# fpgasystems/GPU-FPGA-Recommendation-System

Measured on AMD Instinct MI355X. Metric: inferences/sec at batch 256, higher is better.
Workload: dtype f32; 1 GPU; Model-A (embedding_47_krnl: 47 tables, 1.415 GB) batch=256, fp32 FC 352-1024-512-256-1, all tables resident in one GPU's HBM; hash-filled tables, uniform per-table indices; index rows resident in HBM when the timed region starts (1024 rotating buffers), scores left in HBM (the bench contract's definition of `value`); value_pcie_inclusive = the reference's own loop (cuda_server.c:460-461,494-495): ; batch=256, driver_threads=2, workers_per_thread=2, batches_per_launch=64, parallelism=replicas x1

## Files before the change

gpu-fpga-recommendation-system_amd/csrc/fr_fused.hip:

```cpp
#include "fr_device.h"

#ifdef FR_EPI_FORMS
#include <cstdarg>
#include <cstdio>
thread_local char fr_epi_noted[96];
thread_local int fr_epi_hip_error = 0;
void fr_set_error(const char *, ...) {}
void fr_note_kernel(const char *fmt, ...) {
    va_list ap;
    va_start(ap, fmt);
    vsnprintf(fr_epi_noted, sizeof(fr_epi_noted), fmt, ap);
    va_end(ap);
}
#define FR_NO_DEFAULT_FORM() return FR_ERR_INVALID
#else
static int fused_epi_forward(const FrFusedArgs &a, int kind, hipStream_t s) {
    char name[96] = "";
    const int e = fr_epi_fused_launch(&a, kind, s, name, sizeof(name));
    if (e) FR_FAIL(FR_ERR_HIP, "launch of the epilogue form of the fused kernel failed: %s", hipGetErrorString((hipError_t)e));
    fr_note_kernel("%s", name);
    return FR_OK;
}
#endif

// ... 157 lines not shown
    }
}

template <int NB, int IPT, typename Sink>
__device__ __forceinline__ bool ft_gather_tile(const FrFusedArgs &a, const FrFusedBatch &bt, int m0, int wl, int ig, Sink &&sink) {
    uint64_t base[NB];
    uint32_t stride[NB], rows[NB], icol[NB];
    bool dense[NB];
#pragma unroll
    for (int p = 0; p < NB; p++) {
        const int w = 64 * p + wl < a.n_words ? 64 * p + wl : a.n_words - 1;
        const uint4 d0 = reinterpret_cast<const uint4 *>(a.words)[2 * w];
        const uint4 d1 = reinterpret_cast<const uint4 *>(a.words)[2 * w + 1];
        dense[p] = (d0.w & FR_DESC_DENSE) != 0;
        base[p] = (dense[p] ? (uint64_t)reinterpret_cast<uintptr_t>(bt.dense) : 0ull) + (((uint64_t)d0.y << 32) | d0.x);
        stride[p] = d0.z, rows[p] = d1.x, icol[p] = dense[p] ? 0u : d0.w * 4u;
    }
    const __amdgpu_buffer_rsrc_t rs_idx = __builtin_amdgcn_make_buffer_rsrc(const_cast<int32_t *>(bt.idx), 0, (unsigned)bt.batch * (unsigned)a.idx_stride * 4u, 0x00020000);
    uint32_t id[NB][IPT];
#pragma unroll
    for (int p = 0; p < NB; p++)
#pragma unroll
        for (int i = 0; i < IPT; i++)
            id[p][i] = (uint32_t)__builtin_amdgcn_raw_buffer_load_b32(rs_idx, (unsigned)(m0 + IPT * ig + i) * (unsigned)a.idx_stride * 4u + icol[p], 0, 0);
    bool bad = false;
    uint4 v[NB][IPT];
    auto load_rows = [&](int p) {
#pragma unroll
        for (int i = 0; i < IPT; i++) {
            const unsigned m = (unsigned)(m0 + IPT * ig + i);
            uint32_t r = id[p][i];
            const bool oob = !dense[p] & (r >= rows[p]);
            bad |= oob;
            r = oob ? 0u : r;
            r = dense[p] ? (m < (unsigned)bt.batch ? m : 0u) : r;
            typedef const u32x4_t __attribute__((address_space(1))) * gptr_t;
            const u32x4_t q = *(gptr_t)(base[p] + (uint64_t)r * stride[p]);
            v[p][i] = make_uint4(q.x, q.y, q.z, q.w);
        }
    };
    load_rows(0);
#pragma unroll
    for (int p = 0; p < NB; p++) {
        if (p + 1 < NB) load_rows(p + 1);
        const int w = 64 * p + wl;
        if (w < a.n_words) {
#pragma unroll
            for (int i = 0; i < IPT; i++) sink(w, i, (m0 + IPT * ig + i < bt.batch) ? v[p][i] : make_uint4(0u, 0u, 0u, 0u));
        }
    }
    return bad;
}

template <int T2W, int KG, int WPE, bool DB, bool EPI>
__device__ __forceinline__ void fused_tile_body(const FrFusedArgs &a) {
    extern __shared__ uint4 lds[];
    constexpr int RD = (WPE == 2) ? 1 : 2;
    const int KQ = a.K / 4;
    uint4 *Xq = lds;
    uint4 *R1b[2] = {Xq + (size_t)KQ * FR_FT_LD, Xq + (size_t)(KQ + (DB ? 64 : 0)) * FR_FT_LD};
    uint4 *R2 = lds;
    uint4 *R3 = DB ? lds + (size_t)(a.H2 / 4) * FR_FT_LD : lds;
    const int tid = threadIdx.x, lane = tid & 63;
    const int wave = __builtin_amdgcn_readfirstlane(tid >> 6);
    const int hk = lane >> 5, lm = lane & 31;
    const int bi = blockIdx.x / a.tiles_per_batch, tile = blockIdx.x - bi * a.tiles_per_batch;
    const FrFusedBatch &bt = a.b[bi];
    const int m0 = tile * 32;
    if (m0 >= bt.batch) return;
    int n_st = 0;
    auto stamp = [&]() {
        if (a.stamps && tid == 0 && n_st < 14) {
            a.stamps[16ull * blockIdx.x + n_st] = __builtin_amdgcn_s_memrealtime();
            if (n_st == 1) a.stamps[16ull * blockIdx.x + 14] = __builtin_amdgcn_s_memtime();
            if (n_st == 11) a.stamps[16ull * blockIdx.x + 15] = __builtin_amdgcn_s_memtime();
        }
        n_st++;
    };
    auto wstamp = [&](int k) {
        if (a.stamps && lane == 0) a.stamps[16ull * gridDim.x + (8ull * blockIdx.x + wave) * 4 + k] = __builtin_amdgcn_s_memrealtime();
    };
    stamp();
    const FtW W1 = ft_w(a.w1q, a.K, a.H1, hk, lm), W2 = ft_w(a.w2q, a.H1, a.H2, hk, lm), W3 = ft_w(a.w3q, a.H2, a.H3, hk, lm);
    constexpr int RA = 16 / RD, RB = 24 / T2W / RD;
    constexpr int KG1 = KG > 0 ? KG : 1;
    float4 ring1[RA][1];
    if constexpr (KG > 0) ft_ring_fill<1, RA, KG1>(ring1, W1, 32 * wave, 0);

    if constexpr (KG > 0) {
        const int wl = tid & 63, ig = tid >> 6;
        constexpr int NB = (2 * KG1 + 63) / 64;
        const bool bad = ft_gather_tile<NB, 4>(a, bt, m0, wl, ig, [&](int w, int i, const uint4 &x) { Xq[(size_t)w * FR_FT_LD + 4 * ig + i] = x; });
        if (bad) atomicOr_system(a.err_flag, 1);
    } else {
        const int wl = tid & 63, ig = tid >> 6;
        bool bad = false;
        for (int w0 = 0; w0 < a.n_words; w0 += 64) {
            const int w = w0 + wl;
            if (w < a.n_words) {
                const uint4 d0 = reinterpret_cast<const uint4 *>(a.words)[2 * w];
                const uint4 d1 = reinterpret_cast<const uint4 *>(a.words)[2 * w + 1];
                const uint64_t src = ((uint64_t)d0.y << 32) | d0.x;
                const uint32_t stride = d0.z, idx_col = d0.w, rows = d1.x;
                const bool is_dense = (idx_col & FR_DESC_DENSE) != 0;
                const char *base = is_dense ? reinterpret_cast<const char *>(bt.dense) + src : reinterpret_cast<const char *>(src);
                uint32_t id[4];
#pragma unroll
                for (int i = 0; i < 4; i++) {
                    const int m = m0 + 4 * ig + i;
                    id[i] = 0;
                    if (m < bt.batch) id[i] = is_dense ? (uint32_t)m : (uint32_t)bt.idx[(size_t)m * a.idx_stride + idx_col];
                    if (!is_dense && id[i] >= rows) {
                        bad = true;
                        id[i] = 0;
                    }
                }
                uint4 v[4];
#pragma unroll
                for (int i = 0; i < 4; i++) v[i] = *reinterpret_cast<const uint4 *>(base + (uint64_t)id[i] * stride);
#pragma unroll
                for (int i = 0; i < 4; i++)
                    Xq[(size_t)w * FR_FT_LD + 4 * ig + i] = (m0 + 4 * ig + i < bt.batch) ? v[i] : make_uint4(0u, 0u, 0u, 0u);
            }
        }
        if (bad) atomicOr_system(a.err_flag, 1);
    }
    __syncthreads();
    stamp();

    f32x16 acc2[T2W];
#pragma unroll
    for (int t = 0; t < T2W; t++)
#pragma unroll
        for (int i = 0; i < 16; i++) acc2[t][i] = 0.0f;
    const int n_chunks = a.H1 / 256;
    for (int c = 0; c < n_chunks; c++) {
        f32x16 acc1[1];
#pragma unroll
        for (int i = 0; i < 16; i++) acc1[0][i] = 0.0f;
        if constexpr (KG > 0) ft_gemm_ct<1, RA, KG1>(acc1, ring1, W1, c * 256 + 32 * wave, Xq, 0, 0, hk, lm);
        else ft_gemm<1, 4>(acc1, a.w1q, a.H1, c * 256 + 32 * wave, Xq, 0, 0, a.K / 8, hk, lm);
        stamp();
        if (c == 1) wstamp(0);
        if (c == 2) wstamp(3);
        float4 ring2[RB][T2W];
        ft_ring_fill<T2W, RB, 32>(ring2, W2, 32 * T2W * wave, 32 * c);
        uint4 *R1 = R1b[c & 1];
        if (!DB && c > 0) __syncthreads();
        ft_store_tile<EPI>(R1, acc1[0], 32 * wave, hk, lm, a.epi[0], c * 256 + 32 * wave);
        __syncthreads();
        stamp();
        if (c == 1) wstamp(1);
        ft_gemm_ct<T2W, RB, 32>(acc2, ring2, W2, 32 * T2W * wave, R1, 0, 32 * c, hk, lm);
        if (c == 1) wstamp(2);
        if constexpr (KG > 0) {
            const int cn = (c + 1 < n_chunks) ? c + 1 : c;
            ft_ring_fill<1, RA, KG1>(ring1, W1, cn * 256 + 32 * wave, 0);
        }
    }
    float4 ring3[RA][1];
    ft_ring_fill<1, RA, 32 * T2W>(ring3, W3, 32 * wave, 0);
    __syncthreads();
#pragma unroll
    for (int t = 0; t < T2W; t++) ft_store_tile<EPI>(R2, acc2[t], 32 * (T2W * wave + t), hk, lm, a.epi[1], 32 * (T2W * wave + t));
    __syncthreads();
    stamp();

    f32x16 acc3[1];
#pragma unroll
    for (int i = 0; i < 16; i++) acc3[0][i] = 0.0f;
    ft_gemm_ct<1, RA, 32 * T2W>(acc3, ring3, W3, 32 * wave, R2, 0, 0, hk, lm);
    if (!DB) __syncthreads();
    ft_store_tile<EPI>(R3, acc3[0], 32 * wave, hk, lm, a.epi[2], 32 * wave);
    __syncthreads();
    stamp();
    {
        const int il = tid & 31, sl = tid >> 5;
        const int rows_per = (a.H3 / 4) / 16;
        float s = 0.0f;
        for (int q = sl * rows_per; q < (sl + 1) * rows_per; q++) {
            const uint4 r = R3[(size_t)q * FR_FT_LD + il];
            const float4 w4 = reinterpret_cast<const float4 *>(a.wout)[q];
            s = fmaf(w4.x, __uint_as_float(r.x), s);
            s = fmaf(w4.y, __uint_as_float(r.y), s);
            s = fmaf(w4.z, __uint_as_float(r.z), s);
            s = fmaf(w4.w, __uint_as_float(r.w), s);
        }
        float *part = reinterpret_cast<float *>(R3 + (size_t)64 * FR_FT_LD);
        part[sl * 32 + il] = s;
        __syncthreads();
        if (tid < 32 && m0 + tid < bt.batch) {
            float t = part[tid];
#pragma unroll
            for (int i = 1; i < 16; i++) t += part[i * 32 + tid];
            t = ft_out_bias<EPI>(a, t);
            bt.scores[m0 + tid] = t;
        }
    }
    stamp();
}

#ifndef FR_EPI_FORMS
template <int T2W, int KG, int WPE, bool DB>
__global__ void __launch_bounds__(512, WPE) fr_fused_tile_kernel(const FrFusedArgs a) {
    fused_tile_body<T2W, KG, WPE, DB, false>(a);
}
#else
template <int T2W, int KG, int WPE, bool DB>
__global__ void __launch_bounds__(512, WPE) fr_epi_tile_kernel(const FrFusedArgs a) {
    fused_tile_body<T2W, KG, WPE, DB, true>(a);
}
#endif

size_t frk_fused_lds_bytes(int K, int H2, int wpe) {
    if (wpe == 4) {
        const size_t phase1 = (size_t)(K / 4) + 64, phase2 = (size_t)(H2 / 4) > 68 ? (size_t)(H2 / 4) : 68;
        return (phase1 > phase2 ? phase1 : phase2) * FR_FT_LD * 16;
    }
    const size_t phase1 = (size_t)(K / 4) + 128;
    const size_t phase2 = (size_t)(H2 / 4) + 64 + 4;
    return (phase1 > phase2 ? phase1 : phase2) * FR_FT_LD * 16;
}

bool frk_fused_ok(int K, int H1, int H2, int H3) {
    const bool straight = (K == 352 || K == 880) && H2 == 512;
    if ((!straight && K % 32) || H1 % 256 || (H2 != 256 && H2 != 512) || H3 != 256) return false;
    return frk_fused_lds_bytes(K, H2, 4) <= 160 * 1024;
}

static int fused_wpe(int K, int H2) {
#ifdef FR_EXPERIMENTS
    const int forced = FR_KNOB_ONCE("FUSED_WPE", 0);
    if (forced == 2 || forced == 4) return forced == 4 && frk_fused_lds_bytes(K, H2, 4) > 80 * 1024 ? 2 : forced;
#endif
    return frk_fused_lds_bytes(K, H2, 4) <= 80 * 1024 ? 4 : 2;
}

#ifndef FR_EPI_FORMS
template <int T2W, int KG, int WPE, bool DB>
static int fused_launch_inst(const FrFusedArgs &a, dim3 grid, size_t lds, hipStream_t s) {
    static FrLdsAttrOnce lds_once;
    if (int rc_ = fr_allow_full_lds(&fr_fused_tile_kernel<T2W, KG, WPE, DB>, lds_once)) return rc_;
    fr_fused_tile_kernel<T2W, KG, WPE, DB><<<grid, dim3(512), lds, s>>>(a);
    fr_note_kernel("fr_fused_tile_kernel<%d, %d, %d, %s>", T2W, KG, WPE, DB ? "true" : "false");
    KCHECK();
    return FR_OK;
}

#else
template <int T2W, int KG, int WPE, bool DB>
static int fused_launch_epi_inst(const FrFusedArgs &a, dim3 grid, size_t lds, hipStream_t s) {
    static FrLdsAttrOnce lds_once;
    if (int rc_ = fr_allow_full_lds(&fr_epi_tile_kernel<T2W, KG, WPE, DB>, lds_once)) return rc_;
    fr_epi_tile_kernel<T2W, KG, WPE, DB><<<grid, dim3(512), lds, s>>>(a);
    fr_note_kernel("fr_epi_tile_kernel<%d, %d, %d, %s>", T2W, KG, WPE, DB ? "true" : "false");
    KCHECK();
    return FR_OK;
}

#endif
static bool fused_has_epi(const FrFusedArgs &a) { return a.epi[3].bias != nullptr; }

int frk_fused_launch(const FrFusedArgs &a, hipStream_t s) {
    const int wpe = fused_wpe(a.K, a.H2);
    (void)wpe;
    dim3 grid(a.n_batches * a.tiles_per_batch);
    if (fused_has_epi(a)) {
#ifndef FR_EPI_FORMS
        return fused_epi_forward(a, FR_EPI_KIND_F32, s);
#else
        if (a.H2 == 512 && a.K == 352) return fused_launch_epi_inst<2, 44, 2, true>(a, grid, frk_fused_lds_bytes(a.K, a.H2, 2), s);
        const bool db = frk_fused_lds_bytes(a.K, a.H2, 4) > 80 * 1024 && frk_fused_lds_bytes(a.K, a.H2, 2) <= 160 * 1024;
        const size_t lds = frk_fused_lds_bytes(a.K, a.H2, db ? 2 : 4);
        if (a.H2 == 512) {
            if (a.K == 880) return fused_launch_epi_inst<2, 110, 2, false>(a, grid, lds, s);
            return db ? fused_launch_epi_inst<2, 0, 2, true>(a, grid, lds, s) : fused_launch_epi_inst<2, 0, 2, false>(a, grid, lds, s);
        }
        return db ? fused_launch_epi_inst<1, 0, 2, true>(a, grid, lds, s) : fused_launch_epi_inst<1, 0, 2, false>(a, grid, lds, s);
#endif
    }
#ifdef FR_EPI_FORMS
    FR_NO_DEFAULT_FORM();
#else
    const bool db = wpe == 2 && frk_fused_lds_bytes(a.K, a.H2, 2) <= 160 * 1024;
    const size_t lds = frk_fused_lds_bytes(a.K, a.H2, db ? 2 : 4);
    if (a.H2 == 512) {
        if (a.K == 352) {
#ifdef FR_EXPERIMENTS
            if (wpe != 4) return fused_launch_inst<2, 44, 2, true>(a, grid, lds, s);
#endif
            return fused_launch_inst<2, 44, 4, false>(a, grid, lds, s);
        }
        if (a.K == 880) return fused_launch_inst<2, 110, 2, false>(a, grid, lds, s);
        if (db) return fused_launch_inst<2, 0, 2, true>(a, grid, lds, s);
        return fused_launch_inst<2, 0, 2, false>(a, grid, lds, s);
    }
    if (db) return fused_launch_inst<1, 0, 2, true>(a, grid, lds, s);
    return fused_launch_inst<1, 0, 2, false>(a, grid, lds, s);
#endif
}

constexpr int FR_M2_LD = 65;

template <int NT, int MT, int R, int CNT>
__device__ __forceinline__ void ftm_gemm_ct(f32x16 (&acc)[NT][MT], float4 (&ring)[R][NT], const FtW &w, int n0, const uint4 *Bq, int gb0, int g0, int hk,
                                            int lm) {
    const unsigned s0 = (unsigned)g0 * w.row2 + (unsigned)n0 * 16u;
    const uint4 *bl = Bq + (size_t)(2 * gb0 + hk) * FR_M2_LD + lm;
    uint4 bcur[MT];
#pragma unroll
    for (int mt = 0; mt < MT; mt++) bcur[mt] = bl[32 * mt];
    f32x16 alt[MT];
    if constexpr (NT == 1) {
#pragma unroll
        for (int mt = 0; mt < MT; mt++)
#pragma unroll
            for (int i = 0; i < 16; i++) alt[mt][i] = 0.0f;
    }
#pragma unroll
    for (int g = 0; g < CNT; g++) {
        uint4 bnext[MT];
        const int gn = (g + 1 < CNT) ? g + 1 : g;
#pragma unroll
        for (int mt = 0; mt < MT; mt++) bnext[mt] = bl[(size_t)(2 * gn) * FR_M2_LD + 32 * mt];
        const float4(&a4)[NT] = ring[g % R];
#pragma unroll
        for (int c = 0; c < 4; c++)
#pragma unroll
            for (int t = 0; t < NT; t++)
#pragma unroll
                for (int mt = 0; mt < MT; mt++) {
                    const float av = c == 0 ? a4[t].x : c == 1 ? a4[t].y : c == 2 ? a4[t].z : a4[t].w;
                    const uint32_t bv = c == 0 ? bcur[mt].x : c == 1 ? bcur[mt].y : c == 2 ? bcur[mt].z : bcur[mt].w;
                    if (NT == 1 && (c & 1)) alt[mt] = __builtin_amdgcn_mfma_f32_32x32x2f32(av, __uint_as_float(bv), alt[mt], 0, 0, 0);
                    else acc[t][mt] = __builtin_amdgcn_mfma_f32_32x32x2f32(av, __uint_as_float(bv), acc[t][mt], 0, 0, 0);
                }
        if (g + R < CNT) {
#pragma unroll
            for (int t = 0; t < NT; t++) ring[g % R][t] = ft_wload(w, s0 + (unsigned)(g + R) * w.row2, 512 * t);
        }
        __builtin_amdgcn_sched_barrier(0);
#pragma unroll
        for (int mt = 0; mt < MT; mt++) bcur[mt] = bnext[mt];
    }
    if constexpr (NT == 1) {
#pragma unroll
        for (int mt = 0; mt < MT; mt++)
#pragma unroll
            for (int i = 0; i < 16; i++) acc[0][mt][i] += alt[mt][i];
    }
}

template <bool EPI>
__device__ __forceinline__ void ftm_store_tile(uint4 *img, const f32x16 &acc, int n_local, int m_local, int hk, int lm, const FrEpi &e, int n_glob) {
#pragma unroll
    for (int i = 0; i < 4; i++) {
        float c0 = acc[4 * i + 0], c1 = acc[4 * i + 1], c2 = acc[4 * i + 2], c3 = acc[4 * i + 3];
        ft_epi4<EPI>(c0, c1, c2, c3, e, n_glob + 8 * i, hk);
        uint4 v;
        v.x = __float_as_uint(c0);
        v.y = __float_as_uint(c1);
        v.z = __float_as_uint(c2);
        v.w = __float_as_uint(c3);
        img[(size_t)((n_local >> 2) + 2 * i + hk) * FR_M2_LD + m_local + lm] = v;
    }
}

template <int KG, bool EPI>
__device__ __forceinline__ void fused_tile_m2_body(const FrFusedArgs &a) {
    extern __shared__ uint4 lds[];
    constexpr int LD = FR_M2_LD, MT = 2, T2W = 2, TI = 64;
    constexpr int RA = 12, RB = 8;
    const int KQ = a.K / 4;
    uint4 *Xq = lds;
    uint4 *R1 = Xq + (size_t)KQ * LD;
    uint4 *R2 = lds;
    uint4 *R3 = lds;
    const int tid = threadIdx.x, lane = tid & 63;
    const int wave = __builtin_amdgcn_readfirstlane(tid >> 6);
    const int hk = lane >> 5, lm = lane & 31;
    const int bi = blockIdx.x / a.tiles_per_batch, tile = blockIdx.x - bi * a.tiles_per_batch;
    const FrFusedBatch &bt = a.b[bi];
    const int m0 = tile * TI;
    if (m0 >= bt.batch) return;
    const FtW W1 = ft_w(a.w1q, a.K, a.H1, hk, lm), W2 = ft_w(a.w2q, a.H1, a.H2, hk, lm), W3 = ft_w(a.w3q, a.H2, a.H3, hk, lm);
    float4 ring1[RA][1];
    ft_ring_fill<1, RA, KG>(ring1, W1, 32 * wave, 0);

    {
        const int wl = tid & 63, ig = tid >> 6;
        constexpr int NB = (2 * KG + 63) / 64;
        const bool bad = ft_gather_tile<NB, 8>(a, bt, m0, wl, ig, [&](int w, int i, const uint4 &x) { Xq[(size_t)w * LD + 8 * ig + i] = x; });
        if (bad) atomicOr_system(a.err_flag, 1);
    }
    __syncthreads();

    f32x16 acc2[T2W][MT];
#pragma unroll
    for (int t = 0; t < T2W; t++)
#pragma unroll
        for (int mt = 0; mt < MT; mt++)
#pragma unroll
            for (int i = 0; i < 16; i++) acc2[t][mt][i] = 0.0f;
    const int n_chunks = a.H1 / 256;
    for (int c = 0; c < n_chunks; c++) {
        f32x16 acc1[1][MT];
#pragma unroll
        for (int mt = 0; mt < MT; mt++)
#pragma unroll
            for (int i = 0; i < 16; i++) acc1[0][mt][i] = 0.0f;
        ftm_gemm_ct<1, MT, RA, KG>(acc1, ring1, W1, c * 256 + 32 * wave, Xq, 0, 0, hk, lm);
        float4 ring2[RB][T2W];
        ft_ring_fill<T2W, RB, 32>(ring2, W2, 32 * T2W * wave, 32 * c);
        if (c > 0) __syncthreads();
#pragma unroll
        for (int mt = 0; mt < MT; mt++) ftm_store_tile<EPI>(R1, acc1[0][mt], 32 * wave, 32 * mt, hk, lm, a.epi[0], c * 256 + 32 * wave);
        __syncthreads();
        ftm_gemm_ct<T2W, MT, RB, 32>(acc2, ring2, W2, 32 * T2W * wave, R1, 0, 32 * c, hk, lm);
        const int cn = (c + 1 < n_chunks) ? c + 1 : c;
        ft_ring_fill<1, RA, KG>(ring1, W1, cn * 256 + 32 * wave, 0);
    }
    float4 ring3[RA][1];
    ft_ring_fill<1, RA, 32 * T2W>(ring3, W3, 32 * wave, 0);
    __syncthreads();
#pragma unroll
    for (int t = 0; t < T2W; t++)
#pragma unroll
        for (int mt = 0; mt < MT; mt++) ftm_store_tile<EPI>(R2, acc2[t][mt], 32 * (T2W * wave + t), 32 * mt, hk, lm, a.epi[1], 32 * (T2W * wave + t));
    __syncthreads();

    f32x16 acc3[1][MT];
#pragma unroll
    for (int mt = 0; mt < MT; mt++)
#pragma unroll
        for (int i = 0; i < 16; i++) acc3[0][mt][i] = 0.0f;
    ftm_gemm_ct<1, MT, RA, 32 * T2W>(acc3, ring3, W3, 32 * wave, R2, 0, 0, hk, lm);
    __syncthreads();
#pragma unroll
    for (int mt = 0; mt < MT; mt++) ftm_store_tile<EPI>(R3, acc3[0][mt], 32 * wave, 32 * mt, hk, lm, a.epi[2], 32 * wave);
    __syncthreads();
    {
        const int il = tid & 63, sg = tid >> 6;
        const int rows_per = (a.H3 / 4) / 16;
        float *part = reinterpret_cast<float *>(R3 + (size_t)(a.H3 / 4) * LD);
#pragma unroll
        for (int h2 = 0; h2 < 2; h2++) {
            const int sl = 2 * sg + h2;
            float s = 0.0f;
            for (int q = sl * rows_per; q < (sl + 1) * rows_per; q++) {
                const uint4 r = R3[(size_t)q * LD + il];
                const float4 w4 = reinterpret_cast<const float4 *>(a.wout)[q];
                s = fmaf(w4.x, __uint_as_float(r.x), s);
                s = fmaf(w4.y, __uint_as_float(r.y), s);
                s = fmaf(w4.z, __uint_as_float(r.z), s);
                s = fmaf(w4.w, __uint_as_float(r.w), s);
            }
            part[sl * 64 + il] = s;
        }
        __syncthreads();
        if (tid < 64 && m0 + tid < bt.batch) {
            float t = part[tid];
#pragma unroll
            for (int i = 1; i < 16; i++) t += part[i * 64 + tid];
            t = ft_out_bias<EPI>(a, t);
            bt.scores[m0 + tid] = t;
        }
    }
}

#ifndef FR_EPI_FORMS
template <int KG>
__global__ void __launch_bounds__(512) fr_fused_tile_m2_kernel(const FrFusedArgs a) {
    fused_tile_m2_body<KG, false>(a);
}
#else
template <int KG>
__global__ void __launch_bounds__(512) fr_epi_tile_m2_kernel(const FrFusedArgs a) {
    fused_tile_m2_body<KG, true>(a);
}
#endif

bool frk_fused_m2_ok(int K, int H1, int H2, int H3) { return K == 352 && H1 % 256 == 0 && H2 == 512 && H3 == 256; }

int frk_fused_m2_launch(const FrFusedArgs &a, hipStream_t s) {
    static FrLdsAttrOnce lds_once;
    const size_t rows1 = (size_t)(a.K / 4) + 64, rows2 = (size_t)(a.H2 / 4), rows3 = 64 + 4;
    const size_t rows = rows1 > rows2 ? (rows1 > rows3 ? rows1 : rows3) : (rows2 > rows3 ? rows2 : rows3);
#ifdef FR_EPI_FORMS
    if (!fused_has_epi(a)) FR_NO_DEFAULT_FORM();
    if (int rc_ = fr_allow_full_lds(&fr_epi_tile_m2_kernel<44>, lds_once)) return rc_;
    fr_epi_tile_m2_kernel<44><<<dim3(a.n_batches * a.tiles_per_batch), dim3(512), rows * FR_M2_LD * 16, s>>>(a);
    fr_note_kernel("fr_epi_tile_m2_kernel<44>");
#else
    if (fused_has_epi(a)) return fused_epi_forward(a, FR_EPI_KIND_F32_M2, s);
    if (int rc_ = fr_allow_full_lds(&fr_fused_tile_m2_kernel<44>, lds_once)) return rc_;
    fr_fused_tile_m2_kernel<44><<<dim3(a.n_batches * a.tiles_per_batch), dim3(512), rows * FR_M2_LD * 16, s>>>(a);
    fr_note_kernel("fr_fused_tile_m2_kernel<44>");
#endif
    KCHECK();
    return FR_OK;
}

template <int NT, int MT, int R, int CNT>
__device__ __forceinline__ void fth_gemm_ct(f32x16 (&acc)[NT][MT], const FtW &w, int n0, const uint4 *Bh, int ld, int gb0, int g0, int hk, int lm) {
    const unsigned s0 = (unsigned)g0 * w.row2 + (unsigned)n0 * 16u;
    const uint4 *bl = Bh + (size_t)(2 * gb0 + hk) * ld + lm;
    uint4 ring[R][NT];
#pragma unroll
    for (int g = 0; g < R && g < CNT; g++)
#pragma unroll
        for (int t = 0; t < NT; t++) ring[g][t] = __builtin_bit_cast(uint4, ft_wload(w, s0 + (unsigned)g * w.row2, 512 * t));
#pragma unroll
    for (int g = 0; g < CNT; g++) {
        uint4 b8[MT];
#pragma unroll
        for (int mt = 0; mt < MT; mt++) b8[mt] = bl[(size_t)(2 * g) * ld + 32 * mt];
#pragma unroll
        for (int t = 0; t < NT; t++)
#pragma unroll
            for (int mt = 0; mt < MT; mt++)
                acc[t][mt] = __builtin_amdgcn_mfma_f32_32x32x16_bf16(__builtin_bit_cast(bf16x8, ring[g % R][t]), __builtin_bit_cast(bf16x8, b8[mt]),
                                                                     acc[t][mt], 0, 0, 0);
        if (g + R < CNT) {
#pragma unroll
            for (int t = 0; t < NT; t++) ring[g % R][t] = __builtin_bit_cast(uint4, ft_wload(w, s0 + (unsigned)(g + R) * w.row2, 512 * t));
        }
        __builtin_amdgcn_sched_barrier(0);
    }
}

template <bool EPI>
__device__ __forceinline__ void fth_store_tile(uint4 *img, int ld, const f32x16 &acc, int n_local, int m_local, int hk, int lm, const FrEpi &e, int n_glob) {
    uint2 *h = reinterpret_cast<uint2 *>(img);
#pragma unroll
    for (int i = 0; i < 4; i++) {
        float c0 = acc[4 * i + 0], c1 = acc[4 * i + 1], c2 = acc[4 * i + 2], c3 = acc[4 * i + 3];
        ft_epi4<EPI>(c0, c1, c2, c3, e, n_glob + 8 * i, hk);
        uint2 v;
        v.x = pack_bf16x2(c0, c1);
        v.y = pack_bf16x2(c2, c3);
        h[((size_t)((n_local >> 3) + i) * ld + m_local + lm) * 2 + hk] = v;
    }
}

template <int MT, int T2W, int KG, bool DB, int RD, int PD, bool EPI>
__device__ __forceinline__ void fused_tile_h_body(const FrFusedArgs &a) {
    extern __shared__ uint4 lds[];
    constexpr int LD = 32 * MT + 1, TI = 32 * MT;
    const int KO = a.K / 8;
    uint4 *Xh = lds;
    uint4 *R1b[2] = {Xh + (size_t)KO * LD, Xh + (size_t)(KO + (DB ? 32 : 0)) * LD};
    uint4 *R2 = lds;
    uint4 *R3 = lds + (size_t)(a.H2 / 8) * LD;
    const int tid = threadIdx.x, lane = tid & 63;
    const int wave = __builtin_amdgcn_readfirstlane(tid >> 6);
    const int hk = lane >> 5, lm = lane & 31;
    const int bi = blockIdx.x / a.tiles_per_batch, tile = blockIdx.x - bi * a.tiles_per_batch;
    const FrFusedBatch &bt = a.b[bi];
    const int m0 = tile * TI;
    if (m0 >= bt.batch) return;
    int n_st = 0;
    auto stamp = [&]() {
        if (a.stamps && lane == 0 && n_st < 14) {
            a.stamps[16ull * (8ull * blockIdx.x + wave) + n_st] = __builtin_amdgcn_s_memrealtime();
            if (n_st == 1) a.stamps[16ull * (8ull * blockIdx.x + wave) + 14] = __builtin_amdgcn_s_memtime();
            if (n_st == 9) a.stamps[16ull * (8ull * blockIdx.x + wave) + 15] = __builtin_amdgcn_s_memtime();
        }
        n_st++;
    };
    stamp();

    {
        const int wl = tid & 63, ig = tid >> 6;
        constexpr int IPT = TI / 8, NB = (4 * KG + 63) / 64;
        uint2 *Xh2 = reinterpret_cast<uint2 *>(Xh);
        const bool bad = ft_gather_tile<NB, IPT>(a, bt, m0, wl, ig, [&](int w, int i, const uint4 &x) {
            uint2 hv;
            hv.x = pack_bf16x2(__uint_as_float(x.x), __uint_as_float(x.y));
            hv.y = pack_bf16x2(__uint_as_float(x.z), __uint_as_float(x.w));
            Xh2[((size_t)(w >> 1) * LD + IPT * ig + i) * 2 + (w & 1)] = hv;
        });
        if (bad) atomicOr_system(a.err_flag, 1);
    }
    __syncthreads();
    stamp();

    f32x16 acc2[T2W][MT];
#pragma unroll
    for (int t = 0; t < T2W; t++)
#pragma unroll
        for (int mt = 0; mt < MT; mt++)
#pragma unroll
            for (int i = 0; i < 16; i++) acc2[t][mt][i] = 0.0f;
    const int n_chunks = a.H1 / 256;
    const FtW W1 = ft_w(a.w1q, a.K / 2, a.H1, hk, lm), W2 = ft_w(a.w2q, a.H1 / 2, a.H2, hk, lm), W3 = ft_w(a.w3q, a.H2 / 2, a.H3, hk, lm);
    static_assert(T2W == 2 && KG >= RD && RD >= 8 && RD <= 32 && RD % 2 == 0, "the stream ring assumes two n tiles per wave in FC2 (32 elements per chunk) and at least RD k groups in FC1");
    constexpr int OFF2 = KG % RD;
    uint4 ring[RD];
    auto w1load = [&](int c, int g) { return __builtin_bit_cast(uint4, ft_wload(W1, (unsigned)g * W1.row2 + (unsigned)(c * 256 + 32 * wave) * 16u, 0)); };
    auto w2load = [&](int c, int e) {
        return __builtin_bit_cast(uint4, ft_wload(W2, (unsigned)(16 * c + (e >> 1)) * W2.row2 + (unsigned)(32 * T2W * wave) * 16u, 512 * (e & 1)));
    };
#pragma unroll
    for (int g = 0; g < RD; g++) ring[g] = w1load(0, g);
    const uint4 *blx = Xh + (size_t)hk * LD + lm;
    static_assert(PD == 1 || PD == 2 || PD == 4, "B ring: 16 % PD must be 0");
    uint4 bq[PD][MT];
#pragma unroll
    for (int i = 0; i < PD; i++)
#pragma unroll
        for (int mt = 0; mt < MT; mt++) bq[i][mt] = blx[(size_t)(2 * i) * LD + 32 * mt];
    for (int c = 0; c < n_chunks; c++) {
        f32x16 acc1[1][MT];
#pragma unroll
        for (int mt = 0; mt < MT; mt++)
#pragma unroll
            for (int i = 0; i < 16; i++) acc1[0][mt][i] = 0.0f;
#pragma unroll
        for (int g = 0; g < KG; g++) {
#pragma unroll
            for (int mt = 0; mt < MT; mt++)
                acc1[0][mt] = __builtin_amdgcn_mfma_f32_32x32x16_bf16(__builtin_bit_cast(bf16x8, ring[g % RD]), __builtin_bit_cast(bf16x8, bq[g % PD][mt]), acc1[0][mt], 0, 0, 0);
            if (g + PD < KG) {
#pragma unroll
                for (int mt = 0; mt < MT; mt++) bq[g % PD][mt] = blx[(size_t)(2 * (g + PD)) * LD + 32 * mt];
            }
            if (g + RD < KG) ring[g % RD] = w1load(c, g + RD);
            else ring[g % RD] = w2load(c, (g % RD - OFF2 + RD) % RD);
            __builtin_amdgcn_sched_barrier(0);
        }
        stamp();
        uint4 *R1 = R1b[DB ? (c & 1) : 0];
        if (!DB && c > 0) __syncthreads();
#pragma unroll
        for (int mt = 0; mt < MT; mt++) fth_store_tile<EPI>(R1, LD, acc1[0][mt], 32 * wave, 32 * mt, hk, lm, a.epi[0], c * 256 + 32 * wave);
        __syncthreads();
        const bool last = c + 1 == n_chunks;
        FtW WN = W1;
        if (last) WN = W3;
        const unsigned nsoff = last ? (unsigned)(32 * wave) * 16u : (unsigned)((c + 1) * 256 + 32 * wave) * 16u;
        const uint4 *blr = R1 + (size_t)hk * LD + lm;
#pragma unroll
        for (int i = 0; i < PD; i++)
#pragma unroll
            for (int mt = 0; mt < MT; mt++) bq[i][mt] = blr[(size_t)(2 * i) * LD + 32 * mt];
#pragma unroll
        for (int j = 0; j < 16; j++) {
#pragma unroll
            for (int t = 0; t < T2W; t++)
#pragma unroll
                for (int mt = 0; mt < MT; mt++)
                    acc2[t][mt] = __builtin_amdgcn_mfma_f32_32x32x16_bf16(__builtin_bit_cast(bf16x8, ring[(2 * j + t + OFF2) % RD]), __builtin_bit_cast(bf16x8, bq[j % PD][mt]),
                                                                         acc2[t][mt], 0, 0, 0);
#pragma unroll
            for (int mt = 0; mt < MT; mt++)
                bq[j % PD][mt] = j + PD < 16 ? blr[(size_t)(2 * (j + PD)) * LD + 32 * mt] : blx[(size_t)(2 * (j + PD - 16)) * LD + 32 * mt];
#pragma unroll
            for (int t = 0; t < T2W; t++) {
                const int r = (2 * j + t + OFF2) % RD;
                if (2 * j + t + RD < 32) ring[r] = w2load(c, 2 * j + t + RD);
                else ring[r] = __builtin_bit_cast(uint4, ft_wload(WN, (unsigned)r * WN.row2 + nsoff, 0));
            }
            __builtin_amdgcn_sched_barrier(0);
        }
        stamp();
    }
    __syncthreads();
#pragma unroll
    for (int t = 0; t < T2W; t++)
#pragma unroll
        for (int mt = 0; mt < MT; mt++) fth_store_tile<EPI>(R2, LD, acc2[t][mt], 32 * (T2W * wave + t), 32 * mt, hk, lm, a.epi[1], 32 * (T2W * wave + t));
    __syncthreads();

    f32x16 acc3[1][MT];
#pragma unroll
    for (int mt = 0; mt < MT; mt++)
#pragma unroll
        for (int i = 0; i < 16; i++) acc3[0][mt][i] = 0.0f;
    {
        const uint4 *bl3 = R2 + (size_t)hk * LD + lm;
#pragma unroll
        for (int i = 0; i < PD; i++)
#pragma unroll
            for (int mt = 0; mt < MT; mt++) bq[i][mt] = bl3[(size_t)(2 * i) * LD + 32 * mt];
#pragma unroll
        for (int g = 0; g < 16 * T2W; g++) {
#pragma unroll
            for (int mt = 0; mt < MT; mt++)
                acc3[0][mt] = __builtin_amdgcn_mfma_f32_32x32x16_bf16(__builtin_bit_cast(bf16x8, ring[g % RD]), __builtin_bit_cast(bf16x8, bq[g % PD][mt]), acc3[0][mt], 0, 0, 0);
            if (g + PD < 16 * T2W) {
#pragma unroll
                for (int mt = 0; mt < MT; mt++) bq[g % PD][mt] = bl3[(size_t)(2 * (g + PD)) * LD + 32 * mt];
            }
            if (g + RD < 16 * T2W) ring[g % RD] = __builtin_bit_cast(uint4, ft_wload(W3, (unsigned)(g + RD) * W3.row2 + (unsigned)(32 * wave) * 16u, 0));
            __builtin_amdgcn_sched_barrier(0);
        }
    }
#pragma unroll
    for (int mt = 0; mt < MT; mt++) fth_store_tile<EPI>(R3, LD, acc3[0][mt], 32 * wave, 32 * mt, hk, lm, a.epi[2], 32 * wave);
    __syncthreads();
    stamp();
    {
        const int il = tid % TI, sl = tid / TI;
        constexpr int NSL = 512 / TI;
        const int rows_per = (a.H3 / 8) / NSL;
        const uint4 *wh = reinterpret_cast<const uint4 *>(a.wout);
        float s = 0.0f;
        for (int q = sl * rows_per; q < (sl + 1) * rows_per; q++) {
            const uint4 r = R3[(size_t)q * LD + il];
            const uint4 w = wh[q];
            const uint32_t rr[4] = {r.x, r.y, r.z, r.w}, ww[4] = {w.x, w.y, w.z, w.w};
#pragma unroll
            for (int e = 0; e < 4; e++) {
                s = fmaf(__uint_as_float(ww[e] << 16), __uint_as_float(rr[e] << 16), s);
                s = fmaf(__uint_as_float(ww[e] & 0xFFFF0000u), __uint_as_float(rr[e] & 0xFFFF0000u), s);
            }
        }
        float *part = reinterpret_cast<float *>(R3 + (size_t)(a.H3 / 8) * LD);
        part[sl * TI + il] = s;
        __syncthreads();
        if (tid < TI && m0 + tid < bt.batch) {
            float t = part[tid];
#pragma unroll
            for (int i = 1; i < NSL; i++) t += part[i * TI + tid];
            t = ft_out_bias<EPI>(a, t);
            bt.scores[m0 + tid] = t;
// ... 270 lines not shown
```

Baseline: 69.39 million inferences/s.

## Overlap embedding gather slices with first FC1 chunk in m2 fused kernel

Replaces the up-front embedding gather with three statically cut slices of record words. Only the first slice is written to LDS before FC1 starts. The later slices are loaded and stored to LDS between segments of the first FC1 chunk's K loop, hiding gather latency behind MFMA work. It also reuses the FC1 weight ring to prefetch W3 on the last chunk (non-EPI path), saving a separate ring and refill. The cost is extra barriers, more live registers for the in-flight gather values, and a hard-coded layout for K=352 (88 words).

```diff
diff --git a/gpu-fpga-recommendation-system_amd/csrc/fr_fused.hip b/gpu-fpga-recommendation-system_amd/csrc/fr_fused.hip
--- a/gpu-fpga-recommendation-system_amd/csrc/fr_fused.hip
+++ b/gpu-fpga-recommendation-system_amd/csrc/fr_fused.hip
@@ -483,25 +483,18 @@
 
 constexpr int FR_M2_LD = 65;
 
-template <int NT, int MT, int R, int CNT>
-__device__ __forceinline__ void ftm_gemm_ct(f32x16 (&acc)[NT][MT], float4 (&ring)[R][NT], const FtW &w, int n0, const uint4 *Bq, int gb0, int g0, int hk,
-                                            int lm) {
+template <int NT, int MT, int R, int CNT, int GA, int GB>
+__device__ __forceinline__ void ftm_gemm_seg(f32x16 (&acc)[NT][MT], f32x16 (&alt)[MT], float4 (&ring)[R][NT], const FtW &w, int n0, const uint4 *Bq, int gb0,
+                                             int g0, int hk, int lm) {
     const unsigned s0 = (unsigned)g0 * w.row2 + (unsigned)n0 * 16u;
     const uint4 *bl = Bq + (size_t)(2 * gb0 + hk) * FR_M2_LD + lm;
     uint4 bcur[MT];
 #pragma unroll
-    for (int mt = 0; mt < MT; mt++) bcur[mt] = bl[32 * mt];
-    f32x16 alt[MT];
-    if constexpr (NT == 1) {
-#pragma unroll
-        for (int mt = 0; mt < MT; mt++)
-#pragma unroll
-            for (int i = 0; i < 16; i++) alt[mt][i] = 0.0f;
-    }
-#pragma unroll
-    for (int g = 0; g < CNT; g++) {
+    for (int mt = 0; mt < MT; mt++) bcur[mt] = bl[(size_t)(2 * GA) * FR_M2_LD + 32 * mt];
+#pragma unroll
+    for (int g = GA; g < GB; g++) {
         uint4 bnext[MT];
-        const int gn = (g + 1 < CNT) ? g + 1 : g;
+        const int gn = (g + 1 < GB) ? g + 1 : g;
 #pragma unroll
         for (int mt = 0; mt < MT; mt++) bnext[mt] = bl[(size_t)(2 * gn) * FR_M2_LD + 32 * mt];
         const float4(&a4)[NT] = ring[g % R];
@@ -524,12 +517,34 @@
 #pragma unroll
         for (int mt = 0; mt < MT; mt++) bcur[mt] = bnext[mt];
     }
+}
+
+template <int NT, int MT>
+__device__ __forceinline__ void ftm_alt_zero(f32x16 (&alt)[MT]) {
     if constexpr (NT == 1) {
 #pragma unroll
         for (int mt = 0; mt < MT; mt++)
 #pragma unroll
+            for (int i = 0; i < 16; i++) alt[mt][i] = 0.0f;
+    }
+}
+template <int NT, int MT>
+__device__ __forceinline__ void ftm_alt_add(f32x16 (&acc)[NT][MT], const f32x16 (&alt)[MT]) {
+    if constexpr (NT == 1) {
+#pragma unroll
+        for (int mt = 0; mt < MT; mt++)
+#pragma unroll
             for (int i = 0; i < 16; i++) acc[0][mt][i] += alt[mt][i];
     }
+}
+
+template <int NT, int MT, int R, int CNT>
+__device__ __forceinline__ void ftm_gemm_ct(f32x16 (&acc)[NT][MT], float4 (&ring)[R][NT], const FtW &w, int n0, const uint4 *Bq, int gb0, int g0, int hk,
+                                            int lm) {
+    f32x16 alt[MT];
+    ftm_alt_zero<NT, MT>(alt);
+    ftm_gemm_seg<NT, MT, R, CNT, 0, CNT>(acc, alt, ring, w, n0, Bq, gb0, g0, hk, lm);
+    ftm_alt_add<NT, MT>(acc, alt);
 }
 
 template <bool EPI>
@@ -547,11 +562,79 @@
     }
 }
 
+template <int W0, int W>
+struct FtmSlot {
+    static constexpr int IPT = W / 8;
+    uint64_t base;
+    uint32_t stride, rows, icol;
+    bool dense;
+    uint32_t id[IPT];
+    uint4 v[IPT];
+    static __device__ __forceinline__ int word(int lane) { return W0 + (lane & (W - 1)); }
+    static __device__ __forceinline__ int item(int lane, int wave, int i) { return lane / W + (64 / W) * (wave + 8 * i); }
+    __device__ __forceinline__ void desc(const FrFusedArgs &a, const FrFusedBatch &bt, int lane) {
+        const int w = word(lane) < a.n_words ? word(lane) : a.n_words - 1;
+        const uint4 d0 = reinterpret_cast<const uint4 *>(a.words)[2 * w];
+        const uint4 d1 = reinterpret_cast<const uint4 *>(a.words)[2 * w + 1];
+        dense = (d0.w & FR_DESC_DENSE) != 0;
+        base = (dense ? (uint64_t)reinterpret_cast<uintptr_t>(bt.dense) : 0ull) + (((uint64_t)d0.y << 32) | d0.x);
+        stride = d0.z, rows = d1.x, icol = dense ? 0u : d0.w * 4u;
+    }
+    __device__ __forceinline__ void index(const FrFusedArgs &a, const __amdgpu_buffer_rsrc_t &rs_idx, int m0, int lane, int wave) {
+#pragma unroll
+        for (int i = 0; i < IPT; i++)
+            id[i] = (uint32_t)__builtin_amdgcn_raw_buffer_load_b32(rs_idx, (unsigned)(m0 + item(lane, wave, i)) * (unsigned)a.idx_stride * 4u + icol, 0, 0);
+    }
+    __device__ __forceinline__ bool check(const FrFusedBatch &bt, int m0, int lane, int wave) {
+        bool bad = false;
+#pragma unroll
+        for (int i = 0; i < IPT; i++) {
+            const unsigned m = (unsigned)(m0 + item(lane, wave, i));
+            uint32_t r = id[i];
+            const bool oob = !dense & (r >= rows);
+            bad |= oob;
+            r = oob ? 0u : r;
+            id[i] = dense ? (m < (unsigned)bt.batch ? m : 0u) : r;
+        }
+        return bad;
+    }
+    __device__ __forceinline__ void load() {
+#pragma unroll
+        for (int i = 0; i < IPT; i++) {
+            typedef const u32x4_t __attribute__((address_space(1))) * gptr_t;
+            const u32x4_t q = *(gptr_t)(base + (uint64_t)id[i] * stride);
+            v[i] = make_uint4(q.x, q.y, q.z, q.w);
+        }
+    }
+    __device__ __forceinline__ void put(const FrFusedArgs &a, const FrFusedBatch &bt, uint4 *Xq, int m0, int lane, int wave) const {
+        if (word(lane) < a.n_words) {
+#pragma unroll
+            for (int i = 0; i < IPT; i++) {
+                const int it = item(lane, wave, i);
+                Xq[(size_t)word(lane) * FR_M2_LD + it] = (m0 + it < bt.batch) ? v[i] : make_uint4(0u, 0u, 0u, 0u);
+            }
+        }
+    }
+};
+template <class... S>
+struct FtmSlice : S... {
+    __device__ __forceinline__ void desc(const FrFusedArgs &a, const FrFusedBatch &bt, int lane) { (S::desc(a, bt, lane), ...); }
+    __device__ __forceinline__ void index(const FrFusedArgs &a, const __amdgpu_buffer_rsrc_t &rs, int m0, int lane, int wave) { (S::index(a, rs, m0, lane, wave), ...); }
+    __device__ __forceinline__ bool check(const FrFusedBatch &bt, int m0, int lane, int wave) { return (false | ... | S::check(bt, m0, lane, wave)); }
+    __device__ __forceinline__ void load() { (S::load(), ...); }
+    __device__ __forceinline__ void put(const FrFusedArgs &a, const FrFusedBatch &bt, uint4 *Xq, int m0, int lane, int wave) const { (S::put(a, bt, Xq, m0, lane, wave), ...); }
+};
+constexpr int FR_M2_CUT1 = 12, FR_M2_CUT2 = 28;
+using FtmS0 = FtmSlice<FtmSlot<0, 16>, FtmSlot<16, 8>>;
+using FtmS1 = FtmSlice<FtmSlot<24, 32>>;
+using FtmS2 = FtmSlice<FtmSlot<56, 32>>;
+
 template <int KG, bool EPI>
 __device__ __forceinline__ void fused_tile_m2_body(const FrFusedArgs &a) {
     extern __shared__ uint4 lds[];
     constexpr int LD = FR_M2_LD, MT = 2, T2W = 2, TI = 64;
-    constexpr int RA = 12, RB = 8;
+    constexpr int RA = 12, RB = 8, GC1 = FR_M2_CUT1, GC2 = FR_M2_CUT2;
+    static_assert(KG == 44 && GC1 < GC2 && GC2 < KG, "the slices above are cut for 88 record words");
     const int KQ = a.K / 4;
     uint4 *Xq = lds;
     uint4 *R1 = Xq + (size_t)KQ * LD;
@@ -568,29 +651,21 @@
     float4 ring1[RA][1];
     ft_ring_fill<1, RA, KG>(ring1, W1, 32 * wave, 0);
 
-    {
-        const int wl = tid & 63, ig = tid >> 6;
-        constexpr int NB = (2 * KG + 63) / 64;
-        const bool bad = ft_gather_tile<NB, 8>(a, bt, m0, wl, ig, [&](int w, int i, const uint4 &x) { Xq[(size_t)w * LD + 8 * ig + i] = x; });
-        if (bad) atomicOr_system(a.err_flag, 1);
-    }
-    __syncthreads();
-
+    FtmS0 s0;
+    FtmS1 s1;
+    FtmS2 s2;
+    s0.desc(a, bt, lane), s1.desc(a, bt, lane), s2.desc(a, bt, lane);
+    const __amdgpu_buffer_rsrc_t rs_idx = __builtin_amdgcn_make_buffer_rsrc(const_cast<int32_t *>(bt.idx), 0, (unsigned)bt.batch * (unsigned)a.idx_stride * 4u, 0x00020000);
+    s0.index(a, rs_idx, m0, lane, wave), s1.index(a, rs_idx, m0, lane, wave), s2.index(a, rs_idx, m0, lane, wave);
+    const bool bad0 = s0.check(bt, m0, lane, wave), bad1 = s1.check(bt, m0, lane, wave), bad2 = s2.check(bt, m0, lane, wave);
+    s0.load(), s1.load();
+    if (bad0 | bad1 | bad2) atomicOr_system(a.err_flag, 1);
+    s0.put(a, bt, Xq, m0, lane, wave);
+    __syncthreads();
+
+    const int n_chunks = a.H1 / 256;
     f32x16 acc2[T2W][MT];
-#pragma unroll
-    for (int t = 0; t < T2W; t++)
-#pragma unroll
-        for (int mt = 0; mt < MT; mt++)
-#pragma unroll
-            for (int i = 0; i < 16; i++) acc2[t][mt][i] = 0.0f;
-    const int n_chunks = a.H1 / 256;
-    for (int c = 0; c < n_chunks; c++) {
-        f32x16 acc1[1][MT];
-#pragma unroll
-        for (int mt = 0; mt < MT; mt++)
-#pragma unroll
-            for (int i = 0; i < 16; i++) acc1[0][mt][i] = 0.0f;
-        ftm_gemm_ct<1, MT, RA, KG>(acc1, ring1, W1, c * 256 + 32 * wave, Xq, 0, 0, hk, lm);
+    auto fc2_chunk = [&](int c, f32x16(&acc1)[1][MT]) {
         float4 ring2[RB][T2W];
         ft_ring_fill<T2W, RB, 32>(ring2, W2, 32 * T2W * wave, 32 * c);
         if (c > 0) __syncthreads();
@@ -598,11 +673,49 @@
         for (int mt = 0; mt < MT; mt++) ftm_store_tile<EPI>(R1, acc1[0][mt], 32 * wave, 32 * mt, hk, lm, a.epi[0], c * 256 + 32 * wave);
         __syncthreads();
         ftm_gemm_ct<T2W, MT, RB, 32>(acc2, ring2, W2, 32 * T2W * wave, R1, 0, 32 * c, hk, lm);
-        const int cn = (c + 1 < n_chunks) ? c + 1 : c;
-        ft_ring_fill<1, RA, KG>(ring1, W1, cn * 256 + 32 * wave, 0);
-    }
-    float4 ring3[RA][1];
-    ft_ring_fill<1, RA, 32 * T2W>(ring3, W3, 32 * wave, 0);
+        if constexpr (EPI) {
+            const int cn = (c + 1 < n_chunks) ? c + 1 : c;
+            ft_ring_fill<1, RA, KG>(ring1, W1, cn * 256 + 32 * wave, 0);
+        } else {
+            if (c + 1 < n_chunks) ft_ring_fill<1, RA, KG>(ring1, W1, (c + 1) * 256 + 32 * wave, 0);
+            else ft_ring_fill<1, RA, 32 * T2W>(ring1, W3, 32 * wave, 0);
+        }
+    };
+    {
+        f32x16 acc1[1][MT], alt1[MT];
+#pragma unroll
+        for (int mt = 0; mt < MT; mt++)
+#pragma unroll
+            for (int i = 0; i < 16; i++) acc1[0][mt][i] = 0.0f;
+        ftm_alt_zero<1, MT>(alt1);
+        ftm_gemm_seg<1, MT, RA, KG, 0, GC1>(acc1, alt1, ring1, W1, 32 * wave, Xq, 0, 0, hk, lm);
+        s1.put(a, bt, Xq, m0, lane, wave);
+        __syncthreads();
+        s2.load();
+        ftm_gemm_seg<1, MT, RA, KG, GC1, GC2>(acc1, alt1, ring1, W1, 32 * wave, Xq, 0, 0, hk, lm);
+        s2.put(a, bt, Xq, m0, lane, wave);
+        __syncthreads();
+        ftm_gemm_seg<1, MT, RA, KG, GC2, KG>(acc1, alt1, ring1, W1, 32 * wave, Xq, 0, 0, hk, lm);
+        ftm_alt_add<1, MT>(acc1, alt1);
+#pragma unroll
+        for (int t = 0; t < T2W; t++)
+#pragma unroll
+            for (int mt = 0; mt < MT; mt++)
+#pragma unroll
+                for (int i = 0; i < 16; i++) acc2[t][mt][i] = 0.0f;
+        fc2_chunk(0, acc1);
+    }
+    for (int c = 1; c < n_chunks; c++) {
+        f32x16 acc1[1][MT];
+#pragma unroll
+        for (int mt = 0; mt < MT; mt++)
+#pragma unroll
+            for (int i = 0; i < 16; i++) acc1[0][mt][i] = 0.0f;
+        ftm_gemm_ct<1, MT, RA, KG>(acc1, ring1, W1, c * 256 + 32 * wave, Xq, 0, 0, hk, lm);
+        fc2_chunk(c, acc1);
+    }
+    float4(&ring3)[RA][1] = ring1;
+    if constexpr (EPI) ft_ring_fill<1, RA, 32 * T2W>(ring3, W3, 32 * wave, 0);
     __syncthreads();
 #pragma unroll
     for (int t = 0; t < T2W; t++)
```

Measured after the change: 70.32 million inferences/s (median of 6 runs). +1.3%, better.
